# zkcrypto/bellman

Hardware: AMD Instinct MI355X
Metric: G1 MSM Mscalar-mul/s (BLS12-381, 2^20 bases per GPU) (higher is better)
Workload: dtype u32x12 (381-bit Montgomery integers)

## Files before the change

bellman_amd/_lib.py:

```python

import ctypes
import os
import subprocess

_HERE = os.path.dirname(os.path.abspath(__file__))
_OVERRIDE = os.environ.get("BELLMAN_HIP_LIB") if os.environ.get("BELLMAN_HIP_ALLOW_LIB_OVERRIDE") == "1" else None
LIB_PATH = _OVERRIDE or os.path.join(_HERE, "lib", "libbellman_hip.so")

TEST_LIB_PATH = os.path.join(os.path.dirname(LIB_PATH), "libbellman_hip_test.so")
DEMO_LIB_PATH = os.path.join(os.path.dirname(LIB_PATH), "libbellman_hip_demo.so")
DEMO_EXPORTS = ["bh_groth16_prove_demo", "bh_groth16_demo_r1cs", "bh_groth16_prove_demo_r1cs", "bh_groth16_prove_demo_async",
                "bh_groth16_prove_demo_r1cs_part", "bh_test_synthesis_ms"]

EXPORTS = [
    "bh_version", "bh_ctx_create", "bh_ctx_destroy", "bh_ctx_log_num_cus", "bh_runtime_configure", "bh_ctx_set_limits", "bh_ctx_info",
    "bh_dev_alloc", "bh_dev_free", "bh_dev_upload", "bh_dev_download", "bh_dev_zero", "bh_stream_create", "bh_stream_create_priority", "bh_stream_destroy", "bh_stream_synchronize", "bh_dev_upload_on",
    "bh_dev_zero_on", "bh_ctx_synchronize", "bh_ctx_accumulations_after", "bh_ctx_trim",
    "bh_fft_fr", "bh_fft_fr_dev", "bh_fr_mul_assign_dev", "bh_fr_sub_assign_dev",
    "bh_fr_divide_by_z_on_coset_dev", "bh_fr_distribute_powers_dev", "bh_fft_point_dev", "bh_point_distribute_powers_dev", "bh_point_divide_by_z_on_coset_dev",
    "bh_point_mul_assign_dev", "bh_point_sub_assign_dev", "bh_h_poly_fr", "bh_h_poly_fr_dev", "bh_h_poly_fr_dev_on",
    "bh_bases_register", "bh_bases_register_uncompressed", "bh_bases_read_uncompressed", "bh_bases_read_compressed", "bh_bases_download", "bh_bases_write_uncompressed", "bh_bases_copy_dev", "bh_bases_copy_out_dev", "bh_bases_precompute", "bh_bases_table_info", "bh_bases_wrap_dev", "bh_bases_release", "bh_bases_len",
    "bh_msm_async", "bh_msm_async_dev", "bh_msm_wait", "bh_msm_wait_timed", "bh_msm_wait_profile", "bh_msm_wait_stats", "bh_msm_plan_info", "bh_msm_debug_stages", "bh_point_add", "bh_point_mul", "bh_point_lincomb", "bh_msm_async_opts", "bh_msm_async_dev_opts",
    "bh_scalars_register", "bh_scalars_adopt_dev", "bh_scalars_release", "bh_scalars_len", "bh_scalars_dev_ptr", "bh_msm_async_scalars", "bh_h_poly_fr_scalars", "bh_msm_async_dev_after", "bh_msm_start",
    "bh_msm_sharded_async", "bh_msm_sharded_wait",
    "bh_fixed_base_mul_dev",
    "bh_groth16_params_create", "bh_groth16_params_read", "bh_groth16_generate", "bh_groth16_params_write", "bh_groth16_params_vk_ext", "bh_groth16_params_query", "bh_groth16_params_vk", "bh_proof_write", "bh_groth16_params_release", "bh_groth16_prove_assignment",
    "bh_r1cs_create", "bh_r1cs_release", "bh_r1cs_shape", "bh_r1cs_density", "bh_r1cs_eval_dev", "bh_r1cs_eval_transposed_dev", "bh_fr_powers_dev", "bh_fr_qap_ext_dev",
    "bh_r1cs_eval_transposed_points_dev", "bh_groth16_generate_from_powers_of_tau", "bh_groth16_params_rescale_delta",
    "bh_groth16_prove_witness", "bh_groth16_prove_assignment_async", "bh_groth16_prove_witness_async", "bh_groth16_proof_wait",
    "bh_groth16_prove_witness_part", "bh_groth16_sums_add", "bh_groth16_assemble",
    "bh_groth16_prepare_verifying_key", "bh_groth16_pvk_from_params", "bh_groth16_pvk_num_inputs", "bh_groth16_verify",
    "bh_groth16_batch_verify", "bh_groth16_pvk_release", "bh_proofs_read", "bh_groth16_batch_verify_compressed",
    "bh_groth16_verify_each", "bh_groth16_verify_each_compressed",
]
TEST_EXPORTS = [
    "bh_groth16_prove_demo", "bh_groth16_demo_r1cs", "bh_groth16_prove_demo_r1cs", "bh_groth16_prove_demo_async", "bh_groth16_prove_demo_r1cs_part",
    "bh_test_fr_mul_dev", "bh_test_fp_mul_dev", "bh_test_point_add_dev", "bh_test_g2_k3_dev", "bh_test_g2_pairs_dev", "bh_test_g2_k6_dev",
    "bh_test_fr_mul_host", "bh_test_fr_mul_bform_host", "bh_test_fp_mul_host", "bh_test_point_add_host", "bh_test_point_mul_host", "bh_test_fr_inv_host", "bh_test_fp_lazy_host", "bh_test_proof_slice", "bh_test_synthesis_ms", "bh_test_fr_from_u512_host", "bh_test_fr_ops_host",
    "bh_test_groth16_prove_via_call_sites", "bh_test_demo_assignment", "bh_test_shard_cuts", "bh_test_pool_size_class", "bh_test_capture_check",
    "bh_test_pairing", "bh_test_pairing_host", "bh_test_fp_sqrt_host", "bh_test_fp2_sqrt_host",
    "bh_test_field_ops_shape", "bh_test_field_ops_dev", "bh_test_field_ops_host",
    "bh_test_group_ops_shape", "bh_test_group_ops_dev", "bh_test_group_ops_host", "bh_test_sum_jobs_dev",
    "bh_test_bucket_stage_shape", "bh_test_merge_plan", "bh_test_bucket_stage_dev",
    "bh_test_sort_plan", "bh_test_scan_dev", "bh_test_sort_stage_dev",
    "bh_test_pairing_stage_shape", "bh_test_proof_status_error", "bh_test_pairing_lines_dev", "bh_test_pairing_miller_dev", "bh_test_pairing_fold_dev",
    "bh_test_pairing_proof_prep_dev", "bh_test_pairing_g1_mul_one_dev", "bh_test_pairing_colsum_dev", "bh_test_pairing_ic_table_dev",
    "bh_test_pairing_ic_accumulate_dev", "bh_test_pairing_miller3_dev", "bh_test_pairing_fold3_const_dev",
    "bh_test_pairing_verdict_dev", "bh_test_pairing_final_exp_dev",
]


def library_identity():
    import hashlib

    lib = load()
    with open(LIB_PATH, "rb") as f:
        digest = hashlib.sha256(f.read()).hexdigest()[:16]
    return {"version": lib.bh_version().decode(), "path": os.path.relpath(LIB_PATH, os.path.dirname(_HERE)), "sha256_16": digest,
            "override": bool(_OVERRIDE)}


def build(jobs=8):
    subprocess.check_call(["make", "-C", os.path.join(_HERE, "csrc"), "-j%d" % jobs])
    return LIB_PATH


_lib = None


class _Libs:

    def __init__(self, product, test):
        self.product, self.test = product, test
        self.demo_unchecked = None

    def use_unchecked_demo_circuits(self):
        if self.demo_unchecked is None:
            if not os.path.exists(DEMO_LIB_PATH):
                raise RuntimeError("libbellman_hip_demo.so not built (run `make -C bellman_amd/csrc`)")
            d = ctypes.CDLL(DEMO_LIB_PATH)
            for name in DEMO_EXPORTS:
                f = getattr(d, name)
                t = getattr(self.test, name)
                f.argtypes, f.restype = t.argtypes, t.restype
                self.__dict__[name] = f
            self.demo_unchecked = d
        return self

    def __getattr__(self, name):
        try:
            return getattr(self.product, name)
        except AttributeError:
            if self.test is None:
                raise
            return getattr(self.test, name)


def load():
    global _lib
    if _lib is not None:
        return _lib
    if not os.path.exists(LIB_PATH):
        raise RuntimeError(
            "libbellman_hip.so not built (run `make -C bellman_amd/csrc`); "
            "bellman_amd has no CPU fallback"
        )
    os.environ.setdefault("GPU_MAX_HW_QUEUES", "16")
    product = ctypes.CDLL(LIB_PATH, mode=ctypes.RTLD_GLOBAL)
    lib = _Libs(product, ctypes.CDLL(TEST_LIB_PATH) if os.path.exists(TEST_LIB_PATH) else None)
    lib.bh_runtime_configure()
    c = ctypes
    vp, sz, u32, i32 = c.c_void_p, c.c_size_t, c.c_uint32, c.c_int
    lib.bh_version.restype = c.c_char_p
    lib.bh_ctx_create.argtypes = [i32, c.POINTER(vp)]
    lib.bh_ctx_destroy.argtypes = [vp]
    lib.bh_ctx_destroy.restype = None
    lib.bh_ctx_log_num_cus.argtypes = [vp]
    lib.bh_ctx_log_num_cus.restype = u32
    lib.bh_dev_alloc.argtypes = [vp, sz, c.POINTER(vp)]
    lib.bh_dev_free.argtypes = [vp, vp]
    lib.bh_dev_upload.argtypes = [vp, vp, vp, sz]
    lib.bh_dev_download.argtypes = [vp, vp, vp, sz]
    lib.bh_dev_zero.argtypes = [vp, vp, sz]
    lib.bh_stream_create.argtypes = [vp, c.POINTER(vp)]
    lib.bh_stream_create_priority.argtypes = [vp, i32, c.POINTER(vp)]
    lib.bh_stream_destroy.argtypes = [vp, vp]
# ... 154 lines not shown
```

bellman_amd/csrc/host_fp.hpp:

```cpp
#pragma once
#include <stdint.h>
#include <string.h>
#if defined(__x86_64__) && !defined(__HIP_DEVICE_COMPILE__)
#include <x86intrin.h>
#endif

namespace bh {

struct alignas(16) hfp_t {
  uint64_t l[6];
};
struct alignas(16) hfp2_t {
  hfp_t c0, c1;
};

namespace hostfp {
typedef unsigned __int128 u128;
static const uint64_t MOD[6] = {0xb9feffffffffaaabULL, 0x1eabfffeb153ffffULL, 0x6730d2a0f6b0f624ULL,
                                0x64774b84f38512bfULL, 0x4b1ba7b6434bacd7ULL, 0x1a0111ea397fe69aULL};
static const uint64_t INV = 0x89f3fffcfffcfffdULL;
static const uint64_t ONE[6] = {0x760900000002fffdULL, 0xebf4000bc40c0002ULL, 0x5f48985753c758baULL,
                                0x77ce585370525745ULL, 0x5c071a97a256ec6dULL, 0x15f65ec3fa80e493ULL};

#if defined(__x86_64__) && !defined(__HIP_DEVICE_COMPILE__)
// ... 26 lines not shown
  t[0] = sbb(a.l[0], b.l[0], c); t[1] = sbb(a.l[1], b.l[1], c); t[2] = sbb(a.l[2], b.l[2], c);
  t[3] = sbb(a.l[3], b.l[3], c); t[4] = sbb(a.l[4], b.l[4], c); t[5] = sbb(a.l[5], b.l[5], c);
  const uint64_t m = 0 - (uint64_t)c;
  c = 0;
  r.l[0] = adc(t[0], MOD[0] & m, c); r.l[1] = adc(t[1], MOD[1] & m, c); r.l[2] = adc(t[2], MOD[2] & m, c);
  r.l[3] = adc(t[3], MOD[3] & m, c); r.l[4] = adc(t[4], MOD[4] & m, c); r.l[5] = adc(t[5], MOD[5] & m, c);
}
#if defined(__x86_64__) && defined(__BMI2__) && defined(__ADX__) && !defined(__HIP_DEVICE_COMPILE__)
#define BH_HFP_MULADD(src, tlo, thi) "mulx " src ", %[lo], %[hi]\n\t adcx %[lo], " tlo "\n\t adox %[hi], " thi "\n\t"
#define BH_HFP_ROW(bi)                                                                                               \
  asm("xorl %%eax, %%eax\n\t"                                                                                        \
      BH_HFP_MULADD("%[a0]", "%[t0]", "%[t1]") BH_HFP_MULADD("%[a1]", "%[t1]", "%[t2]")                              \
      BH_HFP_MULADD("%[a2]", "%[t2]", "%[t3]") BH_HFP_MULADD("%[a3]", "%[t3]", "%[t4]")                              \
      BH_HFP_MULADD("%[a4]", "%[t4]", "%[t5]")                                                                       \
      "mulx %[a5], %[lo], %[t6]\n\t adcx %[lo], %[t5]\n\t"                                                           \
      "mov $0, %[lo]\n\t adox %[lo], %[t6]\n\t adcx %[lo], %[t6]\n\t"                                                \
      : [t0] "+r"(t0), [t1] "+r"(t1), [t2] "+r"(t2), [t3] "+r"(t3), [t4] "+r"(t4), [t5] "+r"(t5), [t6] "=&r"(t6),    \
        [lo] "=&r"(lo), [hi] "=&r"(hi)                                                                               \
      : "d"(bi), [a0] "m"(a.l[0]), [a1] "m"(a.l[1]), [a2] "m"(a.l[2]), [a3] "m"(a.l[3]), [a4] "m"(a.l[4]),           \
        [a5] "m"(a.l[5])                                                                                             \
      : "rax", "cc")
#define BH_HFP_REDUCE()                                                                                              \
  {                                                                                                                  \
    const uint64_t m = t0 * INV;                                                                                     \
    asm("xorl %%eax, %%eax\n\t"                                                                                      \
        "mulx %[q0], %[lo], %[hi]\n\t adcx %[t0], %[lo]\n\t adox %[hi], %[t1]\n\t"                                   \
        BH_HFP_MULADD("%[q1]", "%[t1]", "%[t2]") BH_HFP_MULADD("%[q2]", "%[t2]", "%[t3]")                            \
        BH_HFP_MULADD("%[q3]", "%[t3]", "%[t4]") BH_HFP_MULADD("%[q4]", "%[t4]", "%[t5]")                            \
        BH_HFP_MULADD("%[q5]", "%[t5]", "%[t6]")                                                                     \
        "mov $0, %[lo]\n\t adcx %[lo], %[t6]\n\t"                                                                    \
        : [t0] "+r"(t0), [t1] "+r"(t1), [t2] "+r"(t2), [t3] "+r"(t3), [t4] "+r"(t4), [t5] "+r"(t5), [t6] "+r"(t6),   \
          [lo] "=&r"(lo), [hi] "=&r"(hi)                                                                             \
        : "d"(m), [q0] "m"(MOD[0]), [q1] "m"(MOD[1]), [q2] "m"(MOD[2]), [q3] "m"(MOD[3]), [q4] "m"(MOD[4]),          \
          [q5] "m"(MOD[5])                                                                                           \
        : "rax", "cc");                                                                                              \
    t0 = t1; t1 = t2; t2 = t3; t3 = t4; t4 = t5; t5 = t6;                                                            \
  }
static inline void mul(hfp_t &r, const hfp_t &a, const hfp_t &b) {
  uint64_t t0 = 0, t1 = 0, t2 = 0, t3 = 0, t4 = 0, t5 = 0, t6, lo, hi;
  BH_HFP_ROW(b.l[0]); BH_HFP_REDUCE();
  BH_HFP_ROW(b.l[1]); BH_HFP_REDUCE();
  BH_HFP_ROW(b.l[2]); BH_HFP_REDUCE();
  BH_HFP_ROW(b.l[3]); BH_HFP_REDUCE();
  BH_HFP_ROW(b.l[4]); BH_HFP_REDUCE();
  BH_HFP_ROW(b.l[5]); BH_HFP_REDUCE();
  const uint64_t t[6] = {t0, t1, t2, t3, t4, t5};
  final_sub(r.l, t);
}
#undef BH_HFP_MULADD
#undef BH_HFP_ROW
#undef BH_HFP_REDUCE
#else
static inline void mul(hfp_t &r, const hfp_t &a, const hfp_t &b) {
  uint64_t t[8] = {0, 0, 0, 0, 0, 0, 0, 0};
  for (int i = 0; i < 6; i++) {
    u128 c = 0;
    for (int j = 0; j < 6; j++) {
      c += (u128)a.l[j] * b.l[i] + t[j];
      t[j] = (uint64_t)c;
      c >>= 64;
    }
    c += t[6];
    t[6] = (uint64_t)c;
    const uint64_t m = t[0] * INV;
    c = ((u128)m * MOD[0] + t[0]) >> 64;
    for (int j = 1; j < 6; j++) {
      c += (u128)m * MOD[j] + t[j];
      t[j - 1] = (uint64_t)c;
      c >>= 64;
    }
    c += t[6];
    t[5] = (uint64_t)c;
    t[6] = 0;
  }
  final_sub(r.l, t);
}
#endif
static inline bool is_zero(const hfp_t &a) { return (a.l[0] | a.l[1] | a.l[2] | a.l[3] | a.l[4] | a.l[5]) == 0; }
static inline bool eq(const hfp_t &a, const hfp_t &b) {
  uint64_t o = 0;
  for (int i = 0; i < 6; i++) o |= a.l[i] ^ b.l[i];
  return o == 0;
}
static inline void inv(hfp_t &r, const hfp_t &a) {
  uint64_t e[6];
  memcpy(e, MOD, sizeof e);
  e[0] -= 2;
  hfp_t acc;
  memcpy(acc.l, ONE, sizeof ONE);
  for (int i = 383; i >= 0; i--) {
    mul(acc, acc, acc);
    if ((e[i / 64] >> (i % 64)) & 1) mul(acc, acc, a);
  }
  r = acc;
}
}

struct HostFpOps {
  typedef hfp_t T;
  static constexpr bool FUSED_Y3_TAIL = false, FUSED_Y3 = false;
  static void zero(T &r) { memset(&r, 0, sizeof r); }
  static void one(T &r) { memcpy(r.l, hostfp::ONE, sizeof hostfp::ONE); }
  static bool is_zero(const T &a) { return hostfp::is_zero(a); }
  static bool is_zero_canonical(const T &a, const T &b) { return hostfp::is_zero(a) && hostfp::is_zero(b); }
  static bool eq(const T &a, const T &b) { return hostfp::eq(a, b); }
  static void add(T &r, const T &a, const T &b) { hostfp::add(r, a, b); }
  static void sub(T &r, const T &a, const T &b) { hostfp::sub(r, a, b); }
  static void neg(T &r, const T &a) { T z; zero(z); hostfp::sub(r, z, a); }
  static void dbl(T &r, const T &a) { hostfp::add(r, a, a); }
  static void canon(T &) {}
  static void mul(T &r, const T &a, const T &b) { hostfp::mul(r, a, b); }
  static void sqr(T &r, const T &a) { hostfp::mul(r, a, a); }
  static void inv(T &r, const T &a) { hostfp::inv(r, a); }
};

struct HostFp2Ops {
  typedef hfp2_t T;
  typedef HostFpOps B;
  static constexpr bool FUSED_Y3_TAIL = false, FUSED_Y3 = false;
  static void zero(T &r) { memset(&r, 0, sizeof r); }
  static void one(T &r) { B::one(r.c0); B::zero(r.c1); }
  static bool is_zero(const T &a) { return B::is_zero(a.c0) && B::is_zero(a.c1); }
  static bool is_zero_canonical(const T &a, const T &b) { return is_zero(a) && is_zero(b); }
  static bool eq(const T &a, const T &b) { return B::eq(a.c0, b.c0) && B::eq(a.c1, b.c1); }
  static void add(T &r, const T &a, const T &b) { B::add(r.c0, a.c0, b.c0); B::add(r.c1, a.c1, b.c1); }
  static void sub(T &r, const T &a, const T &b) { B::sub(r.c0, a.c0, b.c0); B::sub(r.c1, a.c1, b.c1); }
  static void neg(T &r, const T &a) { B::neg(r.c0, a.c0); B::neg(r.c1, a.c1); }
  static void dbl(T &r, const T &a) { add(r, a, a); }
  static void canon(T &) {}
  static void mul(T &r, const T &a, const T &b) {
    hfp_t t0, t1, t2, t3;
    B::mul(t0, a.c0, b.c0);
    B::mul(t1, a.c1, b.c1);
    B::add(t2, a.c0, a.c1);
    B::add(t3, b.c0, b.c1);
    B::mul(t2, t2, t3);
    B::sub(t2, t2, t0);
    B::sub(r.c1, t2, t1);
    B::sub(r.c0, t0, t1);
  }
  static void sqr(T &r, const T &a) {
    hfp_t s, d, p;
    B::add(s, a.c0, a.c1);
    B::sub(d, a.c0, a.c1);
    B::mul(p, a.c0, a.c1);
    B::mul(r.c0, s, d);
    B::add(r.c1, p, p);
  }
  static void inv(T &r, const T &a) {
    hfp_t n, t;
    B::sqr(n, a.c0);
    B::sqr(t, a.c1);
    B::add(n, n, t);
    B::inv(n, n);
    B::mul(r.c0, a.c0, n);
    B::mul(t, a.c1, n);
    B::neg(r.c1, t);
  }
};

template <class F> struct HostOf;

}
```

bellman_amd/csrc/msm_ec.cuh:

```cuda
#pragma once
#include <string.h>

#include <algorithm>
#include <type_traits>
#include <vector>
#include <cmath>

#include "fp2pair.cuh"
#include "host_fp.hpp"
#include "msm_scalar.cuh"
#include "msm_types.hpp"

namespace bh {

template <class F>
constexpr u32 default_per_wave() { return F::LANES == 3 ? 21u : F::LANES == 2 ? 32u : 64u; }
template <class F>
constexpr u32 tree_per_wave() { return F::LANES == 3 ? 16u : F::LANES == 2 ? 32u : 64u; }
template <class F>
constexpr u32 workers_per_block(u32 threads, u32 per_wave) { return F::LANES == 1 ? threads : (threads / 64u) * per_wave; }

template <class F>
__device__ __forceinline__ u32 worker_role() {
  if constexpr (F::LANES == 1) return 0u;
// ... 1146 lines not shown
      if (force != 2 && (force == 1 || (double)sum_count<FullWK, NW>(js) * 2 <= K2_SUM_FILL * (double)c.num_cus * 4))
        return sum_launch<K2Worker, 1>(js, st);
    }
    if constexpr (std::is_same<FR, Fp2K3Ops>::value) {
      constexpr double K6_SUM_FILL = 8.0;
      SumJobs<M> k6 = js;
      if (force != 2 && (double)sum_count<K6Worker, 4>(k6) <= K6_SUM_FILL * (double)c.num_cus) return sum_launch<K6Worker, 4>(k6, st);
    }
    return sum_launch<FullWK, NW>(js, st);
  };
  {
    const u32 cb = p.c - 1;
    SumDesc dr, dc;
    dr.mode = SUM_STRIDED; dr.groups = p.W * H; dr.count = Lw; dr.inner = H; dr.stride = 1; dr.istride = Lw; dr.group_shift = cb;
    dc = dr; dc.groups = p.W * Lw; dc.count = H; dc.inner = Lw; dc.stride = Lw; dc.istride = 1;
    SumJobs<M> js;
    js.j[0] = make_job(pts, rows, dr); js.j[1] = make_job(pts, cols, dc); js.j[2] = js.j[1]; js.j[2].d.groups = 0;
    if (part) {
      const bool one_lane = G2;
      const u32 len_r = std::min(two_len, Lw), len_c = std::min(two_len, H);
      const u32 Sr = Lw / len_r, Sc = H / len_c;
      Pt *part_r = part, *part_c = part + (u64)dr.groups * Sr;
      SumDesc r1 = dr, c1 = dc;
      r1.splits = Sr; r1.groups = dr.groups * Sr; r1.lanes = 1;
      c1.splits = Sc; c1.groups = dc.groups * Sc; c1.lanes = 1;
      SumJobs<M> s1;
      s1.j[0].in = pts; s1.j[0].out = Sr > 1 ? part_r : rows; s1.j[0].d = r1;
      s1.j[1].in = pts; s1.j[1].out = Sc > 1 ? part_c : cols; s1.j[1].d = c1;
      s1.j[2] = s1.j[1]; s1.j[2].d.groups = 0;
      if (!launch_sums(s1, one_lane ? 2 : 1)) return BH_ERR_HIP;
      SumDesc r2, c2;
      r2.mode = SUM_STRIDED; r2.groups = dr.groups; r2.count = Sr; r2.inner = dr.groups; r2.stride = 1; r2.istride = Sr; r2.group_shift = 0;
      c2 = r2; c2.groups = dc.groups; c2.count = Sc; c2.inner = dc.groups; c2.istride = Sc;
      SumJobs<M> s2;
      s2.j[0] = make_job(part_r, rows, r2); if (Sr <= 1) s2.j[0].d.groups = 0;
      s2.j[1] = make_job(part_c, cols, c2); if (Sc <= 1) s2.j[1].d.groups = 0;
      s2.j[2] = s2.j[1]; s2.j[2].d.groups = 0;
      if (!launch_sums(s2, 1)) return BH_ERR_HIP;
      js.j[0].d.groups = js.j[1].d.groups = 0;
    }
    if (G2 && FR::LANES == 1) {
      const double simds = (double)c.num_cus * 4;
      double best = 1e30;
      u32 best_r = js.j[0].d.lanes, best_c = js.j[1].d.lanes;
      for (u32 gr = 1, lr = 0; gr <= 64 && gr <= std::max(1u, dr.count); gr <<= 1, lr++)
        for (u32 gc = 1, lc = 0; gc <= 64 && gc <= std::max(1u, dc.count); gc <<= 1, lc++) {
          const double steps = std::max((double)((dr.count + gr - 1) / gr) + lr, (double)((dc.count + gc - 1) / gc) + lc);
          const double waves = ((double)dr.groups * gr + (double)dc.groups * gc) / 64.0;
          const double cost = steps * std::max(1.0, waves / simds);
          if (cost < best) { best = cost; best_r = gr; best_c = gc; }
        }
      js.j[0].d.lanes = best_r;
      js.j[1].d.lanes = best_c;
    }
    if (!launch_sums(js)) return BH_ERR_HIP;
    SumDesc bl, bh_, bt;
    bl.mode = SUM_BITS; bl.stride = 1; bl.istride = 0;
    bl.groups = p.W * p.lo_bits; bl.count = Lw; bl.inner = std::max(1u, p.lo_bits); bl.group_shift = p.lo_bits;
    bh_ = bl; bh_.groups = p.W * p.hi_bits; bh_.count = H; bh_.inner = std::max(1u, p.hi_bits); bh_.group_shift = p.hi_bits;
    const bool t_from_cols = Lw < H;
    bt.mode = SUM_STRIDED; bt.groups = p.W; bt.count = t_from_cols ? Lw : H; bt.inner = 1; bt.stride = 1; bt.istride = 0;
    bt.group_shift = t_from_cols ? p.lo_bits : p.hi_bits;
    js.j[0] = make_job(cols, bits, bl);
    js.j[1] = make_job(rows, bits + (u64)p.W * p.lo_bits, bh_);
    js.j[2] = make_job(t_from_cols ? cols : rows, bits + (u64)p.W * cb, bt);
    if (!launch_sums(js)) return BH_ERR_HIP;
  }
  if (job.timed) BH_HIP_CHECK(hipEventRecord(job.ev_end, st));
  job.host_result_bytes = (o_bits - o_err) + bits_bytes;
  if (job.host_result_bytes > job.res.pinned_bytes) return BH_ERR_INVALID_ARG;
  BH_HIP_CHECK(hipMemcpyAsync(job.host_result, ws + o_err, job.host_result_bytes, hipMemcpyDeviceToHost, st));
  return BH_OK;
  };
  if (hold) return BH_OK;
  const int rc2 = job.resume();
  job.resume = nullptr;
  return rc2;
}

template <> struct HostOf<FpOps> { typedef HostFpOps type; };
template <> struct HostOf<Fp2Ops> { typedef HostFp2Ops type; };

template <class F>
static void msm_host_tail(const MsmPlan &p, const XYZZ<F> *bits_dev_layout, void *out_dev_layout) {
  typedef typename HostOf<F>::type H;
  static_assert(sizeof(XYZZ<H>) == sizeof(XYZZ<F>) && sizeof(Affine<H>) == sizeof(Affine<F>), "layout");
  std::vector<XYZZ<F>> canon(bits_dev_layout, bits_dev_layout + (size_t)p.W * p.c);
  for (XYZZ<F> &q : canon) { F::canon(q.x); F::canon(q.y); F::canon(q.zz); F::canon(q.zzz); }
  const XYZZ<H> *bits = reinterpret_cast<const XYZZ<H> *>(canon.data());
  XYZZ<H> acc;
  xyzz_set_identity(acc);
  const u32 cb = p.c - 1;
  const XYZZ<H> *lo = bits, *hi = bits + (size_t)p.W * p.lo_bits, *tot = bits + (size_t)p.W * cb;
  for (int w = (int)p.W - 1; w >= 0; w--) {
    for (int b = (int)p.c - 1; b >= 0; b--) {
      XYZZ<H> t;
      xyzz_dbl(t, acc);
      acc = t;
      if (b < (int)cb) {
        const XYZZ<H> &u = (b >= (int)p.lo_bits) ? hi[(size_t)w * p.hi_bits + (b - p.lo_bits)]
                                                 : lo[(size_t)w * p.lo_bits + b];
        xyzz_add(t, acc, u);
        acc = t;
      }
      if (b == 0) {
        xyzz_add(t, acc, tot[w]);
        acc = t;
      }
    }
  }
  Affine<H> res;
  xyzz_to_affine(res, acc);
  memcpy(out_dev_layout, &res, sizeof res);
}

template <class F>
static int msm_finish(MsmJobImpl &job, void *out_affine, float *ms) {
  Context &c = *job.ctx;
  int rc = BH_OK;
  if (job.trivial) {
    memset(out_affine, 0, sizeof(Affine<F>));
    if (ms) ms[0] = ms[1] = ms[2] = ms[3] = 0.f;
    return job.early_rc;
  }
  if (job.resume) {
    rc = job.resume();
    job.resume = nullptr;
  }
  if (hipStreamSynchronize(job.stream) != hipSuccess) rc = BH_ERR_HIP;
  if (rc == BH_OK) {
    const MsmPlan &p = job.plan;
    constexpr size_t ERR_SLOT = 256;
    ErrFlags ef;
    memcpy(&ef, job.host_result, sizeof ef);
    if (ms) {
      ms[0] = ms[1] = ms[2] = ms[3] = 0.f;
      if (job.timed) {
        (void)hipEventElapsedTime(&ms[0], job.ev_begin, job.ev_end);
        (void)hipEventElapsedTime(&ms[1], job.ev_begin, job.ev_sorted);
        (void)hipEventElapsedTime(&ms[2], job.ev_sorted, job.ev_accum);
        (void)hipEventElapsedTime(&ms[3], job.ev_accum, job.ev_end);
      }
    }
    job.saw_eof = ef.eof != 0;
    job.saw_ident = ef.ident != 0;
    job.done_stats[0] = (u64)p.W * p.n; job.done_stats[1] = ef.zeros; job.done_stats[2] = ef.madds;
    job.done_stats[3] = (u64)p.W * p.chunks_per_window; job.done_stats[4] = p.c; job.done_stats[5] = p.chunk;
    job.done_stats[6] = p.W; job.done_stats[7] = p.Wd;
    if (ef.ident && (ef.eof || job.always_resolve_ident)) {
      const u64 nref = job.ref_n ? job.ref_n : p.nd;
      const double c_ln = (nref < 32) ? 3.0 : std::ceil(std::log((double)nref));
      const u32 c_ref = (u32)c_ln, w_ref = (255 + c_ref - 1) / c_ref, lo_ref = c_ref * (w_ref - 1);
      hipLaunchKernelGGL(msm_err_resolve_kernel<F>, dim3((p.nd + 255) / 256), dim3(256), 0, job.stream,
                         job.scalars_dev, job.fmt, p.nd, job.density_dev, job.word_prefix, job.skip, job.n_bases,
                         (const Affine<F> *)job.bases_dev, job.bases_stride, lo_ref, job.err_dev);
      if (hipMemcpyAsync(&ef, job.err_dev, sizeof ef, hipMemcpyDeviceToHost, job.stream) != hipSuccess ||
          hipStreamSynchronize(job.stream) != hipSuccess)
        rc = BH_ERR_HIP;
      else {
        job.saw_ident_top = ef.ident_top != 0;
        rc = !ef.eof ? BH_ERR_UNEXPECTED_IDENTITY : ef.ident_top ? BH_ERR_UNEXPECTED_IDENTITY : BH_ERR_UNEXPECTED_EOF;
      }
    } else if (ef.eof) {
      rc = BH_ERR_UNEXPECTED_EOF;
    } else if (ef.ident) {
      rc = BH_ERR_UNEXPECTED_IDENTITY;
    } else {
      msm_host_tail<F>(p, (const XYZZ<F> *)((const char *)job.host_result + ERR_SLOT), out_affine);
    }
  }
  for (void *ptr : job.dev_allocs) c.pool.release(ptr);
  job.dev_allocs.clear();
  return rc;
}


template <class F>
static int fixed_base_mul_t(const void *base_host, const void *scalars_dev, u64 n, int fmt, void *out_dev,
                            hipStream_t st, void *table_dev) {
  const u32 blocks = (u32)((n + 127) / 128);
  if (!blocks) return BH_OK;
  Affine<F> b;
  memcpy(&b, base_host, sizeof b);
  Affine<F> *table = (Affine<F> *)table_dev;
  hipLaunchKernelGGL(fixed_base_rows_kernel<F>, dim3(1), dim3(64), 0, st, b, table);
  BH_HIP_CHECK(hipGetLastError());
  hipLaunchKernelGGL(fixed_base_table_kernel<F>, dim3((FB_ROWS * FB_COLS + 127) / 128), dim3(128), 0, st, table);
  BH_HIP_CHECK(hipGetLastError());
  hipLaunchKernelGGL(fixed_base_mul_kernel<F>, dim3(blocks), dim3(128), 0, st, (const Affine<F> *)table, scalars_dev, fmt, n,
                     (Affine<F> *)out_dev);
  BH_HIP_CHECK(hipGetLastError());
  return BH_OK;
}
template <class F>
static int test_point_add_t(void *r, const void *a, const void *b, u64 n, hipStream_t st) {
  const u32 blocks = (u32)((n + 127) / 128);
  if (!blocks) return BH_OK;
  hipLaunchKernelGGL(point_add_kernel<F>, dim3(blocks), dim3(128), 0, st, (Affine<F> *)r, (const Affine<F> *)a,
                     (const Affine<F> *)b, n);
  BH_HIP_CHECK(hipGetLastError());
  return BH_OK;
}
template <class F>
static void generic_point_add(void *r, const void *a, const void *b, u64 n) {
  for (u64 i = 0; i < n; i++) {
    Affine<F> pa, pb, pr;
    memcpy(&pa, (const char *)a + i * sizeof pa, sizeof pa);
    memcpy(&pb, (const char *)b + i * sizeof pb, sizeof pb);
    XYZZ<F> x, y, z;
    xyzz_from_affine(x, pa);
    xyzz_from_affine(y, pb);
    xyzz_add(z, x, y);
    xyzz_to_affine(pr, z);
    memcpy((char *)r + i * sizeof pr, &pr, sizeof pr);
  }
}
template <class F>
static void generic_point_mul(void *r, const void *a, const void *k) {
  Affine<F> base, res;
  u32 kw[8];
  memcpy(&base, a, sizeof base);
  memcpy(kw, k, sizeof kw);
  XYZZ<F> acc;
  xyzz_set_identity(acc);
  for (int b = 255; b >= 0; b--) {
    XYZZ<F> t;
    xyzz_dbl(t, acc);
    acc = t;
    if (((kw[b >> 5] >> (b & 31)) & 1) && !aff_is_identity(base)) xyzz_madd(acc, base);
  }
  xyzz_to_affine(res, acc);
  memcpy(r, &res, sizeof res);
}
template <class F>
static void windowed_point_mul(void *r, const void *a, const u32 *k) {
  Affine<F> base, res;
  memcpy(&base, a, sizeof base);
  u32 kw[9];
  memcpy(kw, k, 32);
  kw[8] = 0;
  bool zero = true;
  for (int i = 0; i < 8; i++) zero &= kw[i] == 0;
  if (aff_is_identity(base) || zero) {
    memset(r, 0, sizeof res);
    return;
  }
  XYZZ<F> tab[8];
  xyzz_from_affine(tab[0], base);
  xyzz_dbl(tab[1], tab[0]);
  for (int i = 2; i < 8; i++) xyzz_add(tab[i], tab[i - 1], tab[0]);
  int digits[65];
// ... 116 lines not shown
```

bellman_amd/csrc/msm_stages.hip:

```cpp
#include <stdlib.h>

#include <algorithm>
#include <cmath>

#include "msm_scalar.cuh"
#include "msm_types.hpp"

namespace bh {

constexpr int SCAN_THREADS = 256;
constexpr int SCAN_PER = 8;
constexpr int SCAN_TILE = SCAN_THREADS * SCAN_PER;

__global__ __launch_bounds__(SCAN_THREADS) void scan_tile_kernel(u32 *data, u32 *block_sums, u64 n) {
  __shared__ u32 wsum[SCAN_THREADS / 64];
  const u32 tid = threadIdx.x, lane = tid & 63, wave = tid >> 6;
  const u64 base = (u64)blockIdx.x * SCAN_TILE + (u64)tid * SCAN_PER;
  u32 v[SCAN_PER];
  u32 run = 0;
#pragma unroll
  for (int k = 0; k < SCAN_PER; k++) {
    u32 t = (base + k < n) ? data[base + k] : 0;
    v[k] = run;
    run += t;
// ... 207 lines not shown
size_t sort_counts_elems(const MsmPlan &p) {
  if (p.W != 1) return (size_t)p.W * 256 * p.num_tiles;
  size_t m = ((size_t)1 << wide_pass_bits(p.c, 0)) * wide_first_tiles(p);
  for (u32 pass = 1; pass < p.sort_passes; pass++) m = std::max(m, ((size_t)1 << wide_pass_bits(p.c, pass)) * p.num_tiles);
  return m;
}

struct WideDigits {
  const void *scalars;
  const u64 *density;
  const u32 *word_prefix;
  u64 skip, n_bases;
  u32 fmt, nd, c, Wd, stride, spt;
};
__device__ __forceinline__ bool wide_load_scalar(const WideDigits &a, u32 i, fr_t &s, u32 &rec, ErrFlags *err) {
  bool dense = true;
  u64 k = a.skip + i;
  if (a.density) {
    const u64 word = a.density[i >> 6];
    dense = (word >> (i & 63)) & 1;
    k = a.skip + a.word_prefix[i >> 6] + __popcll(word & (((u64)1 << (i & 63)) - 1));
  }
  if (!dense) return false;
  if (k >= a.n_bases) {
    if (err) atomicOr(&err->eof, 1u);
    return false;
  }
  load_scalar(a.scalars, i, (int)a.fmt, s);
  rec = (u32)k;
  return true;
}
__device__ __forceinline__ u64 wide_next_digit(fr_t &s, u32 &carry, u32 c) {
  u32 v = (s.l[0] & ((1u << c) - 1)) + carry;
#pragma unroll
  for (int i = 0; i < 7; i++) s.l[i] = (u32)((((u64)s.l[i + 1] << 32) | s.l[i]) >> c);
  s.l[7] >>= c;
  u32 neg = 0;
  carry = 0;
  if (v > (1u << (c - 1))) { v = (1u << c) - v; neg = (v != 0); carry = 1; }
  return ((u64)v << 32) | ((u64)neg << 31);
}
__device__ __forceinline__ u32 wide_bin(u64 entry, u32 shift, u32 bin_mask) { return (((u32)(entry >> 32) - 1u) >> shift) & bin_mask; }

__global__ __launch_bounds__(WIDE_THREADS) void wide_hist_digits_kernel(WideDigits a, u32 *counts, u32 num_tiles, u32 bits,
                                                                        ErrFlags *err) {
  __shared__ u32 hist[WIDE_MAX_BINS];
  const u32 tid = threadIdx.x, tile = blockIdx.x, bins = 1u << bits, bin_mask = bins - 1;
  for (u32 b = tid; b < WIDE_MAX_BINS; b += WIDE_THREADS) hist[b] = 0;
  __syncthreads();
  for (u32 j = 0; j < (u32)WIDE_SCALARS; j++) {
    const u32 local = j * WIDE_THREADS + tid, i = tile * a.spt + local;
    fr_t s;
    u32 rec, carry = 0;
    if (local >= a.spt || i >= a.nd || !wide_load_scalar(a, i, s, rec, err)) continue;
    for (u32 w = 0; w < a.Wd; w++) {
      const u64 e = wide_next_digit(s, carry, a.c);
      if ((u32)(e >> 32)) atomicAdd(&hist[wide_bin(e, 0, bin_mask)], 1u);
    }
  }
  __syncthreads();
  for (u32 b = tid; b < bins; b += WIDE_THREADS) counts[(u64)b * num_tiles + tile] = hist[b];
  if (tile == 0 && tid == 0) counts[(u64)bins * num_tiles] = 0;
}
__global__ __launch_bounds__(WIDE_THREADS) void wide_hist_kernel(const u64 *pairs, u32 *counts, u32 n, u32 shift, u32 bits,
                                                                 u32 num_tiles, const u32 *live_from) {
  __shared__ u32 hist[WIDE_MAX_BINS];
  const u32 tid = threadIdx.x, tile = blockIdx.x, bins = 1u << bits, bin_mask = bins - 1;
  const u32 nn = n - *live_from;
  if (tile * WIDE_TILE >= nn) {
    for (u32 b = tid; b < bins; b += WIDE_THREADS) counts[(u64)b * num_tiles + tile] = 0;
    return;
  }
  for (u32 b = tid; b < WIDE_MAX_BINS; b += WIDE_THREADS) hist[b] = 0;
  __syncthreads();
#pragma unroll 4
  for (int r = 0; r < WIDE_ROUNDS; r++) {
    const u32 idx = tile * WIDE_TILE + r * WIDE_THREADS + tid;
    if (idx < nn) atomicAdd(&hist[wide_bin(pairs[idx], shift, bin_mask)], 1u);
  }
  __syncthreads();
  for (u32 b = tid; b < bins; b += WIDE_THREADS) counts[(u64)b * num_tiles + tile] = hist[b];
}

__global__ void sort_live_kernel(const u32 *scanned_total, u32 *zstart, u32 n) { zstart[0] = n - *scanned_total; }

__device__ __forceinline__ u64 wide_match(u32 bin, bool valid, u32 bits) {
  u64 mask = __ballot(valid);
  for (u32 b = 0; b < bits; b++) {
    const bool bit = (bin >> b) & 1;
    const u64 bal = __ballot(bit);
    mask &= bit ? bal : ~bal;
  }
  return mask;
}

template <bool FUSED>
__global__ __launch_bounds__(WIDE_THREADS) void wide_scatter_kernel(WideDigits a, const u64 *pairs_in, u64 *pairs_out,
                                                                    const u32 *offsets, u32 n, u32 shift, u32 bits,
                                                                    u32 num_tiles, const u32 *live_from, const u32 *out_shift) {
  __shared__ u64 stage[WIDE_TILE];
  __shared__ unsigned short wbase[WIDE_WAVES][WIDE_MAX_BINS];
  __shared__ u32 gbase[WIDE_MAX_BINS];
  __shared__ u32 wsum[WIDE_WAVES];
  u32(*wcnt)[WIDE_MAX_BINS] = reinterpret_cast<u32(*)[WIDE_MAX_BINS]>(stage);
  const u32 tid = threadIdx.x, lane = tid & 63, wave = tid >> 6, tile = blockIdx.x;
  const u32 bins = 1u << bits, bin_mask = bins - 1;
  u32 nn = 0;
  if (!FUSED) {
    nn = n - *live_from;
    if (tile * WIDE_TILE >= nn) return;
  }
  u32 goff[WIDE_BPT];
#pragma unroll
  for (int k = 0; k < WIDE_BPT; k++) goff[k] = tid * WIDE_BPT + k < bins ? offsets[(u64)(tid * WIDE_BPT + k) * num_tiles + tile] : 0;
#pragma unroll
  for (int v = 0; v < WIDE_WAVES; v++)
#pragma unroll
    for (int k = 0; k < WIDE_MAX_BINS / WIDE_THREADS; k++) wcnt[v][k * WIDE_THREADS + tid] = 0;
  __syncthreads();
  if (out_shift) pairs_out += *out_shift;
  const u64 lt_mask = ((u64)1 << lane) - 1;

  fr_t sc[FUSED ? WIDE_SCALARS : 1];
  u32 rec[FUSED ? WIDE_SCALARS : 1];
  bool live[FUSED ? WIDE_SCALARS : 1];
  u64 keys[FUSED ? 1 : WIDE_ROUNDS];
  const u32 first = tile * WIDE_TILE + wave * (WIDE_TILE / WIDE_WAVES) + lane;
  if (FUSED) {
#pragma unroll
    for (int j = 0; j < WIDE_SCALARS; j++) {
      const u32 local = j * WIDE_THREADS + tid, i = tile * a.spt + local;
      live[j] = local < a.spt && i < a.nd && wide_load_scalar(a, i, sc[j], rec[j], nullptr);
    }
  } else {
#pragma unroll
    for (int r = 0; r < WIDE_ROUNDS; r++) keys[r] = first + r * 64 < nn ? pairs_in[first + r * 64] : 0;
  }
  if (FUSED) {
#pragma unroll
    for (int j = 0; j < WIDE_SCALARS; j++) {
      if (!live[j]) continue;
      fr_t s = sc[j];
      u32 carry = 0;
      for (u32 w = 0; w < a.Wd; w++) {
        const u64 e = wide_next_digit(s, carry, a.c);
        if ((u32)(e >> 32)) atomicAdd(&wcnt[wave][wide_bin(e, 0, bin_mask)], 1u);
      }
    }
  } else {
#pragma unroll
    for (int r = 0; r < WIDE_ROUNDS; r++)
      if (first + r * 64 < nn) atomicAdd(&wcnt[wave][wide_bin(keys[r], shift, bin_mask)], 1u);
  }
  __syncthreads();
  u32 cnt[WIDE_BPT][WIDE_WAVES], mine = 0, tile_total = 0;
#pragma unroll
  for (int k = 0; k < WIDE_BPT; k++)
#pragma unroll
    for (int v = 0; v < WIDE_WAVES; v++) { cnt[k][v] = wcnt[v][tid * WIDE_BPT + k]; mine += cnt[k][v]; }
  {
    u32 x = mine;
#pragma unroll
    for (int off = 1; off < 64; off <<= 1) {
      const u32 y = __shfl_up(x, off);
      if (lane >= (u32)off) x += y;
    }
    if (lane == 63) wsum[wave] = x;
    __syncthreads();
    u32 run = x - mine;
#pragma unroll
    for (int v = 0; v < WIDE_WAVES; v++) {
      if ((u32)v < wave) run += wsum[v];
      tile_total += wsum[v];
    }
#pragma unroll
    for (int k = 0; k < WIDE_BPT; k++) {
      gbase[tid * WIDE_BPT + k] = goff[k] - run;
#pragma unroll
      for (int v = 0; v < WIDE_WAVES; v++) { wbase[v][tid * WIDE_BPT + k] = (unsigned short)run; run += cnt[k][v]; }
    }
    __syncthreads();
  }
  auto place = [&](u64 e, bool valid, u32 sh) {
    const u32 bin = wide_bin(e, sh, bin_mask);
    const u64 mask = wide_match(bin, valid, bits);
    const u32 rank = (u32)__popcll(mask & lt_mask);
    u32 pos = 0;
    if (valid) pos = wbase[wave][bin];
    __builtin_amdgcn_wave_barrier();
    if (valid) {
      stage[pos + rank] = e;
      if (rank == 0) wbase[wave][bin] = (unsigned short)(pos + (u32)__popcll(mask));
    }
    __builtin_amdgcn_wave_barrier();
  };
  if (FUSED) {
#pragma unroll
    for (int j = 0; j < WIDE_SCALARS; j++) {
      if (j * WIDE_THREADS + wave * 64 >= a.spt) continue;
      fr_t s = sc[j];
      u32 carry = 0, r = rec[j];
      for (u32 w = 0; w < a.Wd; w++) {
        const u64 e = wide_next_digit(s, carry, a.c) | (r & 0x7fffffffu);
// ... 46 lines not shown
  if (!forced_chunk) p.chunk = (u32)std::max<u64>(p.chunk, (n >> (p.c - 1)) << (p.c >= 20 ? 1 : 0));
  p.chunks_per_window = (p.n + p.chunk - 1) / p.chunk;
  p.sort_passes = (p.c + 7) / 8;
  p.nd = p.n; p.Wd = p.W; p.base_stride = 0;
  return p;
}

unsigned table_window_bits(u64 n_bases, bool g2) {
  const u32 lg = ilog2(n_bases ? n_bases : 1);
  if (g2) return lg <= 10 ? 13 : lg == 11 ? 8 : lg <= 13 ? 10 : 16;
  if (lg <= 10) return 13;
  return lg <= 14 ? 10 : lg <= 18 ? 13 : lg <= 24 ? 20 : 24;
}

MsmPlan make_table_plan(u64 n, const WindowTable &t, unsigned forced_chunk, bool g2, int num_cus) {
  MsmPlan p;
  p.c = t.c;
  p.Wd = (256 + p.c - 1) / p.c;
  p.nd = (u32)n;
  p.base_stride = t.stride;
  p.n = (u32)((u64)p.Wd * n);
  p.W = 1;
  p.nb = 1u << (p.c - 1);
  p.NB = p.nb;
  p.lo_bits = (p.c - 1) / 2;
  p.hi_bits = (p.c - 1) - p.lo_bits;
  p.num_tiles = (p.n + WIDE_TILE - 1) / WIDE_TILE;
  const u32 lg = ilog2(p.n ? p.n : 1);
  const u32 base_k = lg <= 20 ? 8 : lg <= 22 ? 16 : g2 ? 64 : 32;
  const u64 avg = (u64)p.n >> (p.c - 1);
  const u64 lanes_min = (u64)num_cus * 4 * 64 * (g2 ? 1 : 2);
  u64 k = std::max<u64>(base_k, avg);
  k = std::min<u64>(k, std::max<u64>(base_k, (u64)p.n / lanes_min));
  constexpr u64 MIN_ROUNDS = 2;
  if (!g2 && (u64)p.n / lanes_min > k) {
    const u64 per = ((u64)p.n + lanes_min - 1) / lanes_min, rounds = std::max<u64>(MIN_ROUNDS, (per + 127) / 128);
    k = std::max<u64>(k, ((u64)p.n + lanes_min * rounds - 1) / (lanes_min * rounds));
  }
  if (g2 && p.c >= 18 && !forced_chunk) {
    const u64 workers = (u64)num_cus * 4 * 2 * 32;
    const u64 per = ((u64)p.n + workers - 1) / workers, rounds = std::max<u64>(2, (per + 63) / 64);
    k = std::max<u64>(8, ((u64)p.n + workers * rounds - 1) / (workers * rounds));
  }
  p.chunk = forced_chunk ? forced_chunk : (u32)k;
  p.chunks_per_window = (p.n + p.chunk - 1) / p.chunk;
  p.sort_passes = wide_passes(p.c);
  return p;
}


int msm_run_stages(const MsmPlan &p, const MsmBuffers &b, const void *scalars_dev, int fmt, const u64 *density_dev,
                   u64 skip, u64 n_bases, hipStream_t st, const u64 **sorted_out) {
  const u64 n = p.nd;
  const u64 nwords = (n + 63) / 64;
  if (density_dev) {
    hipLaunchKernelGGL(density_popc_kernel, dim3((u32)((nwords + 255) / 256)), dim3(256), 0, st, density_dev,
                       b.word_prefix, nwords);
    BH_HIP_CHECK(hipGetLastError());
    int rc = exclusive_scan_u32(b.word_prefix, nwords, b.scan_tmp, st);
    if (rc) return rc;
  }
  if (p.W == 1) {
    WideDigits a;
    a.scalars = scalars_dev; a.density = density_dev; a.word_prefix = b.word_prefix; a.skip = skip; a.n_bases = n_bases;
    a.fmt = (u32)fmt; a.nd = p.nd; a.c = p.c; a.Wd = p.Wd; a.stride = (u32)p.base_stride; a.spt = wide_scalars_per_tile(p.Wd);
    const u32 tiles0 = wide_first_tiles(p);
    u64 *src = b.pairs_b, *dst = b.pairs_a;
    u32 shift = 0;
    for (u32 pass = 0; pass < p.sort_passes; pass++) {
      const u32 bits = wide_pass_bits(p.c, pass);
      const bool first = pass == 0, last = pass + 1 == p.sort_passes;
      const u32 tiles = first ? tiles0 : p.num_tiles;
      const u64 ncounts = ((u64)1 << bits) * tiles;
      const u32 *out_shift = last ? b.zstart : nullptr;
      if (first)
        hipLaunchKernelGGL(wide_hist_digits_kernel, dim3(tiles), dim3(WIDE_THREADS), 0, st, a, b.counts, tiles, bits, b.err);
      else
        hipLaunchKernelGGL(wide_hist_kernel, dim3(tiles), dim3(WIDE_THREADS), 0, st, src, b.counts, p.n, shift, bits, tiles,
                           b.zstart);
      BH_HIP_CHECK(hipGetLastError());
      int rc = exclusive_scan_u32(b.counts, ncounts + (first ? 1 : 0), b.scan_tmp, st);
      if (rc) return rc;
      if (first) {
        hipLaunchKernelGGL(sort_live_kernel, dim3(1), dim3(1), 0, st, b.counts + ncounts, b.zstart, p.n);
        BH_HIP_CHECK(hipGetLastError());
        hipLaunchKernelGGL(wide_scatter_kernel<true>, dim3(tiles), dim3(WIDE_THREADS), 0, st, a, (const u64 *)nullptr, dst,
                           b.counts, p.n, 0u, bits, tiles, (const u32 *)nullptr, out_shift);
      } else {
        hipLaunchKernelGGL(wide_scatter_kernel<false>, dim3(tiles), dim3(WIDE_THREADS), 0, st, a, src, dst, b.counts, p.n,
                           shift, bits, tiles, b.zstart, out_shift);
      }
      BH_HIP_CHECK(hipGetLastError());
      std::swap(src, dst);
      shift += bits;
    }
    *sorted_out = src;
    return BH_OK;
  }
  hipLaunchKernelGGL(msm_digits_kernel, dim3((p.nd + 255) / 256), dim3(256), 0, st, scalars_dev, fmt, p.nd,
                     density_dev, b.word_prefix, skip, n_bases, p.c, p.Wd, p.base_stride, b.pairs_a, b.err);
  BH_HIP_CHECK(hipGetLastError());
  const u64 ncounts = (u64)p.W * 256 * p.num_tiles;
  u64 *src = b.pairs_a, *dst = b.pairs_b;
  for (u32 pass = 0; pass < p.sort_passes; pass++) {
    const u32 shift = 32 + 8 * pass;
    hipLaunchKernelGGL(sort_hist_kernel, dim3(p.num_tiles, p.W), dim3(SORT_THREADS), 0, st, src, b.counts, p.n,
                       shift, p.num_tiles);
    BH_HIP_CHECK(hipGetLastError());
    int rc = exclusive_scan_u32(b.counts, ncounts, b.scan_tmp, st);
    if (rc) return rc;
    hipLaunchKernelGGL(sort_scatter_kernel, dim3(p.num_tiles, p.W), dim3(SORT_THREADS), 0, st, src, dst, b.counts,
                       p.n, shift, p.num_tiles);
    BH_HIP_CHECK(hipGetLastError());
    std::swap(src, dst);
  }
  *sorted_out = src;
  hipLaunchKernelGGL(window_zero_count_kernel, dim3((p.W + 63) / 64), dim3(64), 0, st, src, b.zstart, p.n, p.W);
  BH_HIP_CHECK(hipGetLastError());
  return BH_OK;
}

}
```

Baseline: 341.5.

## Fold live-count kernel into scatter, use binary GCD host inverse, canon in place

Removes the single-thread sort_live_kernel launch by having the first fused scatter kernel compute the dropped count from the scan total and write it to zstart. The host field inverse switches from Fermat exponentiation to a binary extended Euclid followed by an R^3 Montgomery correction. The host MSM tail now canonicalizes the device result buffer in place instead of copying it into a vector. These trim per-MSM launch and host-tail overhead, at the cost of relying on every tile reading the scan total correctly and on the new inverse being correct.

```diff
diff --git a/bellman_amd/_lib.py b/bellman_amd/_lib.py
--- a/bellman_amd/_lib.py
+++ b/bellman_amd/_lib.py
@@ -41,7 +41,7 @@
     "bh_test_pairing", "bh_test_pairing_host", "bh_test_fp_sqrt_host", "bh_test_fp2_sqrt_host",
     "bh_test_field_ops_shape", "bh_test_field_ops_dev", "bh_test_field_ops_host",
     "bh_test_group_ops_shape", "bh_test_group_ops_dev", "bh_test_group_ops_host", "bh_test_sum_jobs_dev",
-    "bh_test_bucket_stage_shape", "bh_test_merge_plan", "bh_test_bucket_stage_dev",
+    "bh_test_bucket_stage_shape", "bh_test_merge_plan", "bh_test_bucket_stage_dev", "bh_test_fp_inv_host",
     "bh_test_sort_plan", "bh_test_scan_dev", "bh_test_sort_stage_dev",
     "bh_test_pairing_stage_shape", "bh_test_proof_status_error", "bh_test_pairing_lines_dev", "bh_test_pairing_miller_dev", "bh_test_pairing_fold_dev",
     "bh_test_pairing_proof_prep_dev", "bh_test_pairing_g1_mul_one_dev", "bh_test_pairing_colsum_dev", "bh_test_pairing_ic_table_dev",
diff --git a/bellman_amd/csrc/host_fp.hpp b/bellman_amd/csrc/host_fp.hpp
--- a/bellman_amd/csrc/host_fp.hpp
+++ b/bellman_amd/csrc/host_fp.hpp
@@ -132,17 +132,47 @@
   for (int i = 0; i < 6; i++) o |= a.l[i] ^ b.l[i];
   return o == 0;
 }
+static const uint64_t R3[6] = {0xed48ac6bd94ca1e0ULL, 0x315f831e03a7adf8ULL, 0x9a53352a615e29ddULL,
+                               0x34c04e5e921e1761ULL, 0x2512d43565724728ULL, 0x0aa6346091755d4dULL};
+static inline bool geq(const uint64_t *a, const uint64_t *b) {
+  for (int i = 5; i >= 0; i--)
+    if (a[i] != b[i]) return a[i] > b[i];
+  return true;
+}
+static inline bool is_int_one(const uint64_t *a) { return a[0] == 1 && (a[1] | a[2] | a[3] | a[4] | a[5]) == 0; }
+static inline __attribute__((always_inline)) void halve(uint64_t *x) {
+  const uint64_t m = 0 - (x[0] & 1);
+  carry_t c = 0;
+  for (int i = 0; i < 6; i++) x[i] = adc(x[i], MOD[i] & m, c);
+  for (int i = 0; i < 5; i++) x[i] = (x[i] >> 1) | (x[i + 1] << 63);
+  x[5] = (x[5] >> 1) | ((uint64_t)c << 63);
+}
+static inline __attribute__((always_inline)) void shr1(uint64_t *x) {
+  for (int i = 0; i < 5; i++) x[i] = (x[i] >> 1) | (x[i + 1] << 63);
+  x[5] >>= 1;
+}
+static inline __attribute__((always_inline)) void sub_int(uint64_t *r, const uint64_t *b) {
+  carry_t c = 0;
+  for (int i = 0; i < 6; i++) r[i] = sbb(r[i], b[i], c);
+}
 static inline void inv(hfp_t &r, const hfp_t &a) {
-  uint64_t e[6];
-  memcpy(e, MOD, sizeof e);
-  e[0] -= 2;
-  hfp_t acc;
-  memcpy(acc.l, ONE, sizeof ONE);
-  for (int i = 383; i >= 0; i--) {
-    mul(acc, acc, acc);
-    if ((e[i / 64] >> (i % 64)) & 1) mul(acc, acc, a);
-  }
-  r = acc;
+  if (is_zero(a)) { r = a; return; }
+  uint64_t u[6], v[6];
+  hfp_t x1, x2;
+  memcpy(u, a.l, sizeof u);
+  memcpy(v, MOD, sizeof v);
+  memset(&x1, 0, sizeof x1);
+  memset(&x2, 0, sizeof x2);
+  x1.l[0] = 1;
+  while (!is_int_one(u) && !is_int_one(v)) {
+    while (!(u[0] & 1)) { shr1(u); halve(x1.l); }
+    while (!(v[0] & 1)) { shr1(v); halve(x2.l); }
+    if (geq(u, v)) { sub_int(u, v); sub(x1, x1, x2); }
+    else { sub_int(v, u); sub(x2, x2, x1); }
+  }
+  hfp_t r3;
+  memcpy(r3.l, R3, sizeof R3);
+  mul(r, is_int_one(u) ? x1 : x2, r3);
 }
 }
 
diff --git a/bellman_amd/csrc/msm_ec.cuh b/bellman_amd/csrc/msm_ec.cuh
--- a/bellman_amd/csrc/msm_ec.cuh
+++ b/bellman_amd/csrc/msm_ec.cuh
@@ -1252,12 +1252,14 @@
 template <> struct HostOf<Fp2Ops> { typedef HostFp2Ops type; };
 
 template <class F>
-static void msm_host_tail(const MsmPlan &p, const XYZZ<F> *bits_dev_layout, void *out_dev_layout) {
+static void msm_host_tail(const MsmPlan &p, XYZZ<F> *bits_dev_layout, void *out_dev_layout) {
   typedef typename HostOf<F>::type H;
   static_assert(sizeof(XYZZ<H>) == sizeof(XYZZ<F>) && sizeof(Affine<H>) == sizeof(Affine<F>), "layout");
-  std::vector<XYZZ<F>> canon(bits_dev_layout, bits_dev_layout + (size_t)p.W * p.c);
-  for (XYZZ<F> &q : canon) { F::canon(q.x); F::canon(q.y); F::canon(q.zz); F::canon(q.zzz); }
-  const XYZZ<H> *bits = reinterpret_cast<const XYZZ<H> *>(canon.data());
+  for (size_t i = 0; i < (size_t)p.W * p.c; i++) {
+    XYZZ<F> &q = bits_dev_layout[i];
+    F::canon(q.x); F::canon(q.y); F::canon(q.zz); F::canon(q.zzz);
+  }
+  const XYZZ<H> *bits = reinterpret_cast<const XYZZ<H> *>(bits_dev_layout);
   XYZZ<H> acc;
   xyzz_set_identity(acc);
   const u32 cb = p.c - 1;
@@ -1336,7 +1338,7 @@
     } else if (ef.ident) {
       rc = BH_ERR_UNEXPECTED_IDENTITY;
     } else {
-      msm_host_tail<F>(p, (const XYZZ<F> *)((const char *)job.host_result + ERR_SLOT), out_affine);
+      msm_host_tail<F>(p, (XYZZ<F> *)((char *)job.host_result + ERR_SLOT), out_affine);
     }
   }
   for (void *ptr : job.dev_allocs) c.pool.release(ptr);
diff --git a/bellman_amd/csrc/msm_stages.hip b/bellman_amd/csrc/msm_stages.hip
--- a/bellman_amd/csrc/msm_stages.hip
+++ b/bellman_amd/csrc/msm_stages.hip
@@ -313,8 +313,6 @@
   for (u32 b = tid; b < bins; b += WIDE_THREADS) counts[(u64)b * num_tiles + tile] = hist[b];
 }
 
-__global__ void sort_live_kernel(const u32 *scanned_total, u32 *zstart, u32 n) { zstart[0] = n - *scanned_total; }
-
 __device__ __forceinline__ u64 wide_match(u32 bin, bool valid, u32 bits) {
   u64 mask = __ballot(valid);
   for (u32 b = 0; b < bits; b++) {
@@ -328,7 +326,8 @@
 template <bool FUSED>
 __global__ __launch_bounds__(WIDE_THREADS) void wide_scatter_kernel(WideDigits a, const u64 *pairs_in, u64 *pairs_out,
                                                                     const u32 *offsets, u32 n, u32 shift, u32 bits,
-                                                                    u32 num_tiles, const u32 *live_from, const u32 *out_shift) {
+                                                                    u32 num_tiles, const u32 *live_from, const u32 *out_shift,
+                                                                    u32 *live_out) {
   __shared__ u64 stage[WIDE_TILE];
   __shared__ unsigned short wbase[WIDE_WAVES][WIDE_MAX_BINS];
   __shared__ u32 gbase[WIDE_MAX_BINS];
@@ -349,7 +348,13 @@
 #pragma unroll
     for (int k = 0; k < WIDE_MAX_BINS / WIDE_THREADS; k++) wcnt[v][k * WIDE_THREADS + tid] = 0;
   __syncthreads();
-  if (out_shift) pairs_out += *out_shift;
+  if (FUSED) {
+    const u32 dropped = n - offsets[(u64)bins * num_tiles];
+    if (tile == 0 && tid == 0) *live_out = dropped;
+    if (out_shift) pairs_out += dropped;
+  } else if (out_shift) {
+    pairs_out += *out_shift;
+  }
   const u64 lt_mask = ((u64)1 << lane) - 1;
 
   fr_t sc[FUSED ? WIDE_SCALARS : 1];
@@ -562,13 +567,11 @@
       int rc = exclusive_scan_u32(b.counts, ncounts + (first ? 1 : 0), b.scan_tmp, st);
       if (rc) return rc;
       if (first) {
-        hipLaunchKernelGGL(sort_live_kernel, dim3(1), dim3(1), 0, st, b.counts + ncounts, b.zstart, p.n);
-        BH_HIP_CHECK(hipGetLastError());
         hipLaunchKernelGGL(wide_scatter_kernel<true>, dim3(tiles), dim3(WIDE_THREADS), 0, st, a, (const u64 *)nullptr, dst,
-                           b.counts, p.n, 0u, bits, tiles, (const u32 *)nullptr, out_shift);
+                           b.counts, p.n, 0u, bits, tiles, (const u32 *)nullptr, out_shift, b.zstart);
       } else {
         hipLaunchKernelGGL(wide_scatter_kernel<false>, dim3(tiles), dim3(WIDE_THREADS), 0, st, a, src, dst, b.counts, p.n,
-                           shift, bits, tiles, b.zstart, out_shift);
+                           shift, bits, tiles, b.zstart, out_shift, (u32 *)nullptr);
       }
       BH_HIP_CHECK(hipGetLastError());
       std::swap(src, dst);
```

Measured after the change: 344.6, median of 6. About the same (+0.9%).
